# hannesweisbach/channelcoding

Measured on AMD Instinct MI355X. Metric: decoded frames/sec (coded bits/sec = value x 255), BCH(255,231) min-sum, batch=2^20, higher is better.
Workload: dtype f32

## Files before the change

channelcoding_amd/csrc/cc_internal.hpp:

```cpp
#pragma once
#include <hip/hip_runtime.h>

#include <cstdint>
#include <memory>
#include <mutex>
#include <string>
#include <vector>

#include "../../include/channelcoding_amd.h"
#include "galois.hpp"

namespace ccamd {

struct MinSumGeometry {
  int W = 64, C = 4, frames_per_wave = 1, KW = 1;
};

struct MinSumParams {
  int n, K, KW;
  int variant;
  int stop_rule;
  unsigned iterations;
  float alpha_f;
  float beta_f;
// ... 41 lines not shown
  uint32_t root_log[64] = {0};
  uint32_t n = 0, k = 0, l = 0, t = 0, nroots = 0, q = 0;
  uint32_t nf = 0;
  int family = 0;
};

}

namespace ccamd {
struct McWorkspace;
void mc_workspace_free(McWorkspace *w);
struct HostStage;
void host_stage_free(HostStage *s);
}

struct cc_code {
  cc_desc desc;
  int device = 0;
  std::unique_ptr<ccamd::Field> field;
  ccamd::CodeTables tab;
  bool wide = false;
  std::unique_ptr<ccamd::FieldT<uint16_t>> field16;
  ccamd::CodeTablesT<uint16_t> tab16;
  ccamd::WideTables wide_dev;
  uint16_t *d_wide = nullptr;
  bool soft = false;
  std::vector<uint8_t> custom_H;
  bool matrix_only = false;
  unsigned ms_rows = 0;
  ccamd::MinSumGeometry geo;
  uint32_t *d_colmask = nullptr;
  uint16_t *d_diag = nullptr;
  uint32_t *d_colbits = nullptr;
  uint8_t *d_parity = nullptr;
  ccamd::AlgebraicTables *d_alg = nullptr;
  ccamd::AlgebraicTables h_alg;
  mutable ccamd::McWorkspace *mc = nullptr;
  mutable ccamd::HostStage *stage = nullptr;
  mutable std::mutex lazy_lock;
  hipMemPool_t pool = nullptr;
  int num_cus = 256;
  bool force_generic = false;
  std::string name;
  bool shortened = false;
  unsigned long long *d_osd_rows = nullptr;
};

namespace ccamd {

inline bool rs_twisted(const cc_code *code) {
  return code->tab.family == CC_FAMILY_RS && (code->desc.mu != 1 || code->desc.step != 1);
}

inline hipError_t workspace_alloc(const cc_code *code, void **p, size_t bytes, hipStream_t stream) {
  return code->pool ? hipMallocFromPoolAsync(p, bytes, code->pool, stream) : hipMallocAsync(p, bytes, stream);
}

struct Scratch {
  const cc_code *code;
  hipStream_t stream;
  void *p[6] = {nullptr, nullptr, nullptr, nullptr, nullptr, nullptr};
  int used = 0;
  Scratch(const cc_code *c, hipStream_t s) : code(c), stream(s) {}
  Scratch(const Scratch &) = delete;
  Scratch &operator=(const Scratch &) = delete;
  ~Scratch() {
    for (int i = 0; i < used; ++i)
      if (p[i]) (void)hipFreeAsync(p[i], stream);
  }
  template <class T>
  hipError_t get(T **out, size_t bytes) {
    const hipError_t e = workspace_alloc(code, &p[used], bytes ? bytes : 1, stream);
    *out = static_cast<T *>(p[used]);
    if (e == hipSuccess) ++used;
    return e;
  }
};

void set_last_error(const std::string &s);
int hip_fail(hipError_t e, const char *what);

#define CC_HIP_TRY(expr)                                   \
  do {                                                     \
    hipError_t _e = (expr);                                \
    if (_e != hipSuccess) return ccamd::hip_fail(_e, #expr); \
  } while (0)

int launch_minsum(const cc_code *code, const float *d_llr, const uint16_t *d_er, const uint32_t *d_er_off,
                  uint8_t *d_hard, float *d_L, uint16_t *d_iters, int32_t *d_status, size_t B, hipStream_t stream);
struct DiagGeometry {
  unsigned n, k, w;
  int D, LPF, CPL;
  bool scms;
  int np = 0;
  int gap[4] = {0, 0, 0, 0};
};
const DiagGeometry *diag_geometry(const CodeTables &t);
std::vector<uint16_t> build_diag_table(const CodeTables &t, int D, int W, int np = 0, const int *gap = nullptr);
size_t minsum_diag_lds_bytes(const DiagGeometry &g);
MinSumParams minsum_params(const cc_code *code);
bool minsum_shortcuts_enabled();
bool minsum_diag_supported(const cc_code *code);
int launch_minsum_diag_compact(const cc_code *code, uint32_t *d_ctl, uint32_t *d_pool, unsigned cap, const float *d_llr,
                               uint8_t *d_hard, uint16_t *d_iters, int32_t *d_status, hipStream_t stream);
std::string minsum_diag_name(const cc_code *code);
int launch_minsum_diag(const cc_code *code, const MinSumParams &p, const float *d_llr, const uint16_t *d_er,
                       const uint32_t *d_er_off, uint8_t *d_hard, float *d_L, uint16_t *d_iters, int32_t *d_status,
                       size_t B, hipStream_t stream);
bool algebraic_long_needed(const cc_code *code, bool erasures);
int launch_algebraic_long(const cc_code *code, bool float_in, const void *d_in, const uint16_t *d_er,
                          const uint32_t *d_er_off, uint8_t *d_out, int32_t *d_nerr, int32_t *d_status, size_t B,
                          hipStream_t stream);
int launch_algebraic(const cc_code *code, bool float_in, const void *d_in, const uint16_t *d_er,
                     const uint32_t *d_er_off, uint8_t *d_out, int32_t *d_nerr, int32_t *d_status, size_t B,
                     hipStream_t stream);
bool algebraic_chunk_supported(const cc_code *code, bool erasures);
int launch_algebraic_chunk(const cc_code *code, bool float_in, const void *d_in, const uint16_t *d_er,
                           const uint32_t *d_er_off, uint8_t *d_out, int32_t *d_nerr, int32_t *d_status, size_t B,
                           hipStream_t stream, int il = 1);
int launch_chase(const cc_code *code, const float *d_llr, unsigned p, uint8_t *d_out, int32_t *d_nerr, float *d_metric,
                 int32_t *d_status, size_t B, hipStream_t stream);
int chase_frames_per_wave(const cc_code *code, unsigned p, bool soft, bool extended = false);
int launch_chase_soft(const cc_code *code, const float *d_llr, unsigned p, float beta, uint8_t *d_out, float *d_ext,
                      int32_t *d_nerr, float *d_metric, int32_t *d_status, size_t B, hipStream_t stream);
int launch_chase_extended(const cc_code *code, const float *d_llr, unsigned p, float beta, uint8_t *d_out, float *d_ext,
                          int32_t *d_nerr, float *d_metric, int32_t *d_status, size_t B, hipStream_t stream);
int launch_osd(const cc_code *code, const float *d_llr, unsigned order, uint8_t *d_out, int32_t *d_nerr, float *d_metric,
               int32_t *d_status, size_t B, hipStream_t stream);
int osd_frames_per_wave(const cc_code *code);
std::vector<unsigned long long> build_osd_rows(const CodeTables &t);
int launch_gmd(const cc_code *code, const uint8_t *d_words, const float *d_rel, unsigned m, uint8_t *d_out, int32_t *d_nerr,
               float *d_metric, int32_t *d_status, size_t B, hipStream_t stream);
bool bitslice_supported(const cc_code *code);
int launch_bitslice_syndromes(const cc_code *code, bool float_in, const void *d_in, uint8_t *d_out, uint8_t *d_synd, size_t B,
                              hipStream_t stream, int il = 1);
bool bitslice_encode_supported(const cc_code *code);
int launch_bitslice_encode(const cc_code *code, const uint8_t *d_msg, uint8_t *d_cw, size_t B, hipStream_t stream, int il = 1);
int launch_bitslice_chien(const void *d_lamp, void *d_masks, size_t B, bool long_locators, hipStream_t stream);
int launch_bitslice_roots_transpose(const void *d_masks, void *d_rootsT, size_t B, hipStream_t stream);
constexpr uint32_t kLogZero = 512;
int launch_chunk_bm(const cc_code *code, const uint8_t *d_synd, const uint16_t *d_er, const uint32_t *d_er_off,
                    uint16_t *d_llg, uint16_t *d_meta, unsigned long long *d_mask, uint8_t *d_lamp, int ncoef,
                    uint32_t *d_nleft, int32_t *d_nerr, int32_t *d_status, size_t B, hipStream_t stream);
int algebraic_route(const cc_code *code, size_t B, bool erasures);
bool planes_small_call(const cc_code *code, size_t B);
int launch_pgz_erasures(const cc_code *code, const uint8_t *d_in, const uint16_t *d_er, const uint32_t *d_er_off,
                        uint8_t *d_out, int32_t *d_nerr, int32_t *d_status, size_t B, hipStream_t stream);
constexpr int diag_variant_part(int variant, int parts) {
  const int order = variant == CC_ALG_MS ? 0 : variant == CC_ALG_NMS ? 1 : variant == CC_ALG_OMS ? 2
                  : variant == CC_ALG_SCMS2 ? 3 : variant == CC_ALG_SCMS1 ? 4 : 5;
  return order % parts;
}

enum DiagRowBody { DIAG_ROWS_BUTTERFLY = 0, DIAG_ROWS_FOUR = 1, DIAG_ROWS_FOUR_PIPELINED = 2 };
#ifndef CC_DIAG_FOUR_ROW_BODY
#define CC_DIAG_FOUR_ROW_BODY 1
#endif
constexpr int diag_row_body(int K, int D, int LPF, int variant) {
  const bool plain = variant == CC_ALG_MS || variant == CC_ALG_NMS || variant == CC_ALG_OMS || variant == CC_ALG_2DNMS;
  return (K == 24 && D == 7 && LPF == 16 && plain) ? CC_DIAG_FOUR_ROW_BODY : DIAG_ROWS_BUTTERFLY;
}

int launch_wide_correct(const cc_code *code, const uint16_t *d_in, const uint16_t *d_er, const uint32_t *d_off,
                        uint16_t *d_out, int32_t *d_nerr, int32_t *d_status, size_t B, hipStream_t stream);
int launch_wide_pgz_erasures(const cc_code *code, const uint16_t *d_in, const uint16_t *d_er, const uint32_t *d_off,
                        uint16_t *d_out, int32_t *d_nerr, int32_t *d_status, size_t B, hipStream_t stream);
int launch_wide_encode(const cc_code *code, const uint16_t *d_msg, uint16_t *d_cw, size_t B, hipStream_t stream);
int launch_wide_extract(const cc_code *code, const uint16_t *d_cw, uint16_t *d_msg, size_t B, hipStream_t stream);
std::vector<uint8_t> build_parity_table(const Field &f, const CodeTables &t);
int launch_encode(const cc_code *code, const uint8_t *d_msg, uint8_t *d_cw, size_t B, hipStream_t stream);
int launch_encode_bits(const cc_code *code, const uint8_t *d_msg, uint8_t *d_cw, size_t B, hipStream_t stream);
int launch_extract(const cc_code *code, const uint8_t *d_cw, uint8_t *d_msg, size_t B, hipStream_t stream);
int launch_pack_bits(const void *d_sym, int width, size_t n, uint8_t *d_packed, size_t B, hipStream_t stream);
int launch_unpack_bits(const uint8_t *d_packed, size_t n, void *d_sym, int width, size_t B, hipStream_t stream);
bool packed_native_supported(const cc_code *code, size_t B);
int launch_packed_correct(const cc_code *code, const uint8_t *d_in, uint8_t *d_out, int32_t *d_nerr, int32_t *d_status,
                          size_t B, hipStream_t stream);
bool packed_long_supported(const cc_code *code, size_t B);
int launch_packed_long_correct(const cc_code *code, const uint8_t *d_in, uint8_t *d_out, int32_t *d_nerr, int32_t *d_status,
                               size_t B, hipStream_t stream);
bool packed_encode_native(const cc_code *code);
bool packed_extract_native(const cc_code *code);
int launch_packed_encode(const cc_code *code, const uint8_t *d_msg, uint8_t *d_cw, size_t B, hipStream_t stream);
int launch_packed_extract(const cc_code *code, const uint8_t *d_cw, uint8_t *d_msg, size_t B, hipStream_t stream);
constexpr size_t kInterleaveMax = 256;
constexpr size_t kInterleaveNativeMax = 16;
int launch_interleave(const void *d_in, int width, size_t n, size_t I, void *d_out, size_t B, bool to_interleaved,
                      hipStream_t stream);
bool interleaved_native_supported(const cc_code *code, size_t B, size_t I, bool erasures);
bool interleaved_encode_native(const cc_code *code, size_t I);
bool interleaved_extract_native(const cc_code *code, size_t I);
int launch_interleaved_extract(const cc_code *code, const void *d_cw, void *d_msg, size_t B, size_t I, hipStream_t stream);
struct ProductShape {
  int e;
  size_t w1, w2, k1, k2, N;
};
ProductShape product_shape(const cc_product *pc);
size_t product_chunk_blocks(size_t N, size_t blocks, size_t at_least = 1);
int launch_product_decode(const cc_product *pc, const float *d_y, uint8_t *d_out, float *d_ext, int32_t *d_status, size_t B,
                          hipStream_t stream);
int launch_product_encode(const cc_product *pc, const uint8_t *d_msg, uint8_t *d_cw, size_t B, hipStream_t stream);
int launch_product_extract(const cc_product *pc, const uint8_t *d_cw, uint8_t *d_msg, size_t B, hipStream_t stream);
int product_awgn(const cc_product *pc, double ebno_db, uint64_t seed, uint64_t first_block, size_t blocks,
                 int random_codewords, float *d_y, uint8_t *d_sent, hipStream_t stream);
int mc_run_product(const cc_product *pc, double ebno_db, uint64_t seed, uint64_t first_block, size_t blocks,
                   int random_codewords, uint64_t *d_counters, hipStream_t stream);
int mc_run_product_hard(const cc_product *pc, double ebno_db, uint64_t seed, uint64_t first_block, size_t blocks,
                        int random_codewords, uint64_t *d_counters, hipStream_t stream);
int launch_product_hard(const cc_product *pc, const uint8_t *d_in, uint8_t *d_out, int32_t *d_nflip, int32_t *d_last,
                        int32_t *d_status, size_t B, hipStream_t stream);
struct StaircaseShape {
  int e;
  size_t m, r, kb, L, N, K;
};
StaircaseShape staircase_shape(const cc_staircase *sc);
size_t staircase_lds_bytes(const cc_staircase *sc);
int launch_staircase_decode(const cc_staircase *sc, const uint8_t *d_in, uint8_t *d_out, int32_t *d_nflip, int32_t *d_status,
                            size_t B, hipStream_t stream);
int launch_staircase_encode(const cc_staircase *sc, const uint8_t *d_msg, uint8_t *d_cw, size_t B, hipStream_t stream);
int launch_staircase_extract(const cc_staircase *sc, const uint8_t *d_cw, uint8_t *d_msg, size_t B, hipStream_t stream);
int staircase_awgn(const cc_staircase *sc, double ebno_db, uint64_t seed, uint64_t first_stream, size_t streams,
                   int random_codewords, uint8_t *d_z, uint8_t *d_sent, hipStream_t stream);
int mc_run_staircase(const cc_staircase *sc, double ebno_db, uint64_t seed, uint64_t first_stream, size_t streams,
                     int random_codewords, uint64_t *d_counters, hipStream_t stream);
int mc_run(cc_code *code, double ebno_db, uint64_t seed, uint64_t first_frame, size_t frames, int random_codewords,
           uint64_t *d_counters, hipStream_t stream);
int mc_run_chase(cc_code *code, unsigned p, double ebno_db, uint64_t seed, uint64_t first_frame, size_t frames,
                 int random_codewords, uint64_t *d_counters, hipStream_t stream);
int mc_run_osd(cc_code *code, unsigned order, double ebno_db, uint64_t seed, uint64_t first_frame, size_t frames,
               int random_codewords, uint64_t *d_counters, hipStream_t stream);
int mc_run_gmd(cc_code *code, unsigned m, double ebno_db, uint64_t seed, uint64_t first_frame, size_t frames,
               int random_codewords, uint64_t *d_counters, hipStream_t stream);
int mc_awgn_symbols(cc_code *code, double ebno_db, uint64_t seed, uint64_t first_frame, size_t frames, int random_codewords,
                    uint8_t *d_words, float *d_rel, uint8_t *d_sent, hipStream_t stream);
int mc_awgn(cc_code *code, double ebno_db, uint64_t seed, uint64_t first_frame, size_t frames, int random_codewords,
            float *d_llr, uint8_t *d_sent, hipStream_t stream);
int launch_awgn_values(const cc_code *code, int n, float sigma, uint64_t seed, uint64_t first_frame, size_t frames,
                       float *d_llr, const uint8_t *sent, hipStream_t stream, unsigned long long *d_counters = nullptr);
int launch_awgn_hard(const cc_code *code, int n, float sigma, uint64_t seed, uint64_t first_frame, size_t frames,
                     uint8_t *d_hard, const uint8_t *sent, hipStream_t stream, unsigned long long *d_counters = nullptr);
int launch_random_bits(const cc_code *code, int l, uint64_t seed, uint64_t first_frame, size_t frames, uint8_t *d_msg,
                       hipStream_t stream);
int mc_run_discrete(cc_code *code, double p_error, double p_erasure, uint64_t seed, uint64_t first_frame, size_t frames,
                    int random_codewords, uint64_t *d_counters, hipStream_t stream);
int mc_discrete(cc_code *code, double p_error, double p_erasure, uint64_t seed, uint64_t first_frame, size_t frames,
                int random_codewords, uint8_t *d_recv, uint16_t *d_erasures, uint32_t *d_erasure_offsets,
                uint8_t *d_sent, hipStream_t stream);
int mc_run_burst(cc_code *code, const cc_burst_channel &ch, uint64_t seed, uint64_t first_frame, size_t frames,
                 int random_codewords, uint64_t *d_counters, hipStream_t stream);
int mc_burst(cc_code *code, const cc_burst_channel &ch, uint64_t seed, uint64_t first_frame, size_t frames,
             int random_codewords, uint8_t *d_recv, uint8_t *d_sent, uint8_t *d_state, hipStream_t stream);
int mc_run_burst_erasure(cc_code *code, const cc_burst_channel &ch, const cc_burst_detector &det, uint64_t seed,
                         uint64_t first_frame, size_t frames, int random_codewords, uint64_t *d_counters,
                         hipStream_t stream);
int mc_burst_erasure(cc_code *code, const cc_burst_channel &ch, const cc_burst_detector &det, uint64_t seed,
                     uint64_t first_frame, size_t frames, int random_codewords, uint8_t *d_recv, uint8_t *d_sent,
                     uint8_t *d_state, uint8_t *d_flag, uint16_t *d_erasures, uint32_t *d_erasure_offsets,
                     hipStream_t stream);
int mc_run_bsc_packed(cc_code *code, double p_error, uint64_t seed, uint64_t first_frame, size_t frames,
                      int random_codewords, uint64_t *d_counters, hipStream_t stream);
int mc_bsc_packed(cc_code *code, double p_error, uint64_t seed, uint64_t first_frame, size_t frames, int random_codewords,
                  uint8_t *d_recv, uint8_t *d_sent, hipStream_t stream);
int launch_bsc_packed(const cc_code *code, unsigned long long threshold, uint64_t seed, uint64_t first_frame, size_t frames,
                      const uint8_t *d_sent, uint8_t *d_recv, unsigned long long *d_counters, hipStream_t stream);
int launch_random_packed_messages(const cc_code *code, uint64_t seed, uint64_t first_frame, size_t frames, uint8_t *d_msg,
                                  hipStream_t stream);
int launch_count_packed(const cc_code *code, const uint8_t *d_decoded, const uint8_t *d_sent, const int32_t *d_status,
                        size_t frames, unsigned long long *d_counters, hipStream_t stream);
int packed_correct_route(const cc_code *code, const uint8_t *d_in, uint8_t *d_out, int32_t *d_nerr, int32_t *d_status,
                         size_t B, hipStream_t stream);
int packed_encode_route(const cc_code *code, const uint8_t *d_msg, uint8_t *d_cw, size_t B, hipStream_t stream);
int minsum_kernel_info(const cc_code *code, std::string &name, uint32_t &frames_per_wg, uint32_t &threads,
                       uint32_t &lds);

}
```

channelcoding_amd/csrc/minsum_diag.hip:

```cpp
#include "minsum_diag_impl.hpp"

#include <algorithm>
#include <cstdlib>

namespace ccamd {

using DiagLaunch = int (*)(const cc_code *, const MinSumParams &, const float *, const uint16_t *, const uint32_t *,
                           uint8_t *, float *, uint16_t *, int32_t *, size_t, hipStream_t);
#define CC_PART_DECL(NAME, I)                                                                                        \
  int launch_minsum_diag_##NAME##_p##I(const cc_code *, const MinSumParams &, const float *, const uint16_t *,       \
                                       const uint32_t *, uint8_t *, float *, uint16_t *, int32_t *, size_t, hipStream_t);
#define CC_PARTS_1(M, NAME) M(NAME, 0)
#define CC_PARTS_2(M, NAME) CC_PARTS_1(M, NAME) M(NAME, 1)
#define CC_PARTS_3(M, NAME) CC_PARTS_2(M, NAME) M(NAME, 2)
#define CC_PARTS_6(M, NAME) CC_PARTS_3(M, NAME) M(NAME, 3) M(NAME, 4) M(NAME, 5)
#define GEO(NAME, N, KK, W, DD, LL, CC, OO, SC, PA, LK, PP) CC_PARTS_##PP(CC_PART_DECL, NAME)
#include "minsum_diag_geos.inc"
#undef GEO
namespace {
struct DiagEntry {
  DiagGeometry geo;
  int parts;
  DiagLaunch launch[6];
};
// ... 41 lines not shown
    bool ok = true;
    for (int p = 0; p < np && ok; ++p) {
      std::vector<unsigned> c;
      for (unsigned s : sup)
        if (in_sup[s + gap[p]]) c.push_back(s);
      for (size_t i = c.size(); i > 1; --i) std::swap(c[i - 1], c[next() % i]);
      bool res[16] = {false};
      for (int pass = 0; pass < 2 && low[p].size() < static_cast<size_t>(W); ++pass)
        for (unsigned s : c) {
          if (used[s] || used[s + gap[p]] || (pass == 0 && res[s % 16])) continue;
          used[s] = used[s + gap[p]] = 1;
          res[s % 16] = true;
          low[p].push_back(s);
          if (low[p].size() == static_cast<size_t>(W)) break;
        }
      ok = low[p].size() == static_cast<size_t>(W);
    }
    if (!ok) continue;
    std::vector<unsigned> single;
    for (unsigned s : sup)
      if (!used[s]) single.push_back(s);
    int cost = 0;
    for (int p = 0; p < np; ++p) cost += passes(low[p]);
    {
      int cnt[16] = {0}, mx = 0;
      for (unsigned s : single) mx = std::max(mx, ++cnt[s % 16]);
      cost += std::max(singles_per_lane, mx);
    }
    if (cost < best_cost) {
      best_cost = cost;
      best_low = low;
      best_single = single;
    }
  }
  if (best_cost == 1 << 30) return {};
  std::vector<uint16_t> out(static_cast<size_t>(D) * W, 0xFFFFu);
  for (int p = 0; p < np; ++p) {
    std::sort(best_low[p].begin(), best_low[p].end());
    for (int l = 0; l < W; ++l) {
      out[(2 * p) * W + l] = static_cast<uint16_t>(best_low[p][l]);
      out[(2 * p + 1) * W + l] = static_cast<uint16_t>(best_low[p][l] + gap[p]);
    }
  }
  std::vector<std::vector<unsigned>> cls(16);
  for (unsigned s : best_single) cls[s % 16].push_back(s);
  std::vector<std::vector<unsigned>> slot(singles_per_lane);
  int turn = 0;
  for (int r = 0; r < 16; ++r)
    for (unsigned s : cls[r]) {
      int tries = 0;
      while (slot[turn % singles_per_lane].size() >= static_cast<size_t>(W) && tries++ < singles_per_lane) ++turn;
      slot[turn++ % singles_per_lane].push_back(s);
    }
  for (int g = 0; g < singles_per_lane; ++g)
    for (size_t l = 0; l < slot[g].size(); ++l) out[(2 * np + g) * W + l] = static_cast<uint16_t>(slot[g][l]);
  return out;
}

std::vector<uint16_t> build_diag_table(const CodeTables &t, int D, int W, int np, const int *gap) {
#ifdef CC_AMD_EXPERIMENTS
  if (const char *e = std::getenv("CC_AMD_EXP_FAKE_DEAL"); e && e[0] == '1') {
    std::vector<uint16_t> out(static_cast<size_t>(D) * W);
    for (int d = 0; d < D; ++d)
      for (int l = 0; l < W; ++l)
        out[d * W + l] = static_cast<uint16_t>(d < 2 * np ? l + W * (d & ~1) + (d & 1) : l + W * d);
    return out;
  }
#endif
  if (np > 0) return build_paired_table(t, D, W, np, gap);
  std::vector<std::vector<unsigned>> cls(W);
  for (unsigned s : t.row0_support) cls[s % W].push_back(s);
  std::vector<std::vector<unsigned>> grp(D);
  std::vector<unsigned> left;
  for (int r = 0; r < W; ++r)
    for (size_t e = 0; e < cls[r].size(); ++e) {
      if (e < static_cast<size_t>(D))
        grp[e].push_back(cls[r][e]);
      else
        left.push_back(cls[r][e]);
    }
  for (int g = 0; g < D; ++g) {
    while (grp[g].size() < static_cast<size_t>(W) && !left.empty()) {
      size_t best = 0;
      int best_mult = 1 << 30;
      for (size_t c = 0; c < left.size(); ++c) {
        int mult = 1;
        for (unsigned s : grp[g]) mult += (s % W == left[c] % W);
        if (mult < best_mult) {
          best_mult = mult;
          best = c;
        }
      }
      grp[g].push_back(left[best]);
      left.erase(left.begin() + static_cast<long>(best));
    }
  }
  for (int g = 0; g + 1 < D; ++g)
    while (grp[g].size() < static_cast<size_t>(W) && !grp[D - 1].empty()) {
      grp[g].push_back(grp[D - 1].back());
      grp[D - 1].pop_back();
    }
  const size_t real_last = grp[D - 1].size();
  auto group_cost = [&](const std::vector<unsigned> &g) {
    int cnt[16] = {0}, mx = 0, sq = 0;
    for (unsigned s : g) ++cnt[s % 16];
    for (int c : cnt) {
      mx = c > mx ? c : mx;
      sq += c * c;
    }
    return mx * 1000 + sq;
  };
  bool improved = true;
  while (improved) {
    improved = false;
    for (int a = 0; a < D && !improved; ++a)
      for (int b = a + 1; b < D && !improved; ++b)
        for (size_t x = 0; x < grp[a].size() && !improved; ++x)
          for (size_t y = 0; y < grp[b].size() && !improved; ++y) {
            const int before = group_cost(grp[a]) + group_cost(grp[b]);
            std::swap(grp[a][x], grp[b][y]);
            if (group_cost(grp[a]) + group_cost(grp[b]) < before)
              improved = true;
            else
              std::swap(grp[a][x], grp[b][y]);
          }
  }
  std::vector<uint16_t> out(static_cast<size_t>(D) * W, 0xFFFFu);
  for (int g = 0; g < D; ++g)
    for (size_t l = 0; l < grp[g].size(); ++l) out[g * W + l] = static_cast<uint16_t>(grp[g][l]);
  (void)real_last;
  return out;
}

bool minsum_diag_supported(const cc_code *code) {
  if (code->d_diag == nullptr || code->desc.iterations == 0) return false;
  const int alg = code->desc.algorithm;
  const DiagGeometry *geo = diag_geometry(code->tab);
  if (!geo) return false;
  if (alg == CC_ALG_SCMS1) return true;
  if (alg == CC_ALG_SCMS2) return geo->scms;
  if (alg != CC_ALG_MS && alg != CC_ALG_NMS && alg != CC_ALG_OMS && alg != CC_ALG_2DNMS) return false;
  if (alg == CC_ALG_OMS && !(code->desc.beta >= 0.0)) return false;
  const float a = static_cast<float>(code->desc.alpha);
  if ((alg == CC_ALG_NMS || alg == CC_ALG_2DNMS) && !(a == a && a - a == 0.0f)) return false;
  return diag_geometry(code->tab) != nullptr;
}


std::string minsum_diag_name(const cc_code *code) {
  const DiagGeometry *g = diag_geometry(code->tab);
  if (!g) return "minsum_diag_kernel";
  const int body = diag_row_body(static_cast<int>(g->k), g->D, g->LPF, code->desc.algorithm);
  return "minsum_diag_kernel<K=" + std::to_string(g->k) + ",D=" + std::to_string(g->D) + ",LPF=" + std::to_string(g->LPF) +
         (body == DIAG_ROWS_FOUR_PIPELINED ? ",four-row-pipelined>" : body == DIAG_ROWS_FOUR ? ",four-row>" : ",row-pipelined>");
}

size_t minsum_diag_lds_bytes(const DiagGeometry &g) {
  const bool partial = g.w != static_cast<unsigned>(g.LPF * g.D);
  const size_t fpw = 64 / g.LPF, rc = static_cast<size_t>(g.LPF) * g.CPL + (partial ? 48 : (g.LPF == 8 && g.CPL == 8 ? 8 : 16));
  return 4 * (fpw * rc * 8 + (fpw / 2) * rc * 8) + 256 * 4 +
         4 * static_cast<size_t>(g.CPL) * 256;
}


namespace {

__global__ void __launch_bounds__(256)
twopass_gather_kernel(const uint32_t *__restrict__ ctl, unsigned sample, unsigned cap, const uint32_t *__restrict__ list,
                      const float *__restrict__ llr, float *__restrict__ llr2, int n) {
  if (!two_pass_in_effect(ctl, sample, cap)) return;
  const unsigned long long cnt = ctl[1];
  const int lane = threadIdx.x & 63;
  const unsigned long long nwaves = static_cast<unsigned long long>(gridDim.x) * 4;
  for (unsigned long long k = static_cast<unsigned long long>(blockIdx.x) * 4 + (threadIdx.x >> 6); k < cnt; k += nwaves) {
    const float *src = llr + static_cast<unsigned long long>(list[k]) * n;
    float *dst = llr2 + k * n;
    for (int j = lane; j < n; j += 64) dst[j] = src[j];
  }
}
__global__ void __launch_bounds__(256)
twopass_scatter_kernel(const uint32_t *__restrict__ ctl, unsigned sample, unsigned cap, const uint32_t *__restrict__ list,
                       const uint8_t *__restrict__ hard2, const uint16_t *__restrict__ iters2,
                       const int32_t *__restrict__ status2, uint8_t *__restrict__ hard, uint16_t *__restrict__ iters,
                       int32_t *__restrict__ status, int n) {
  if (!two_pass_in_effect(ctl, sample, cap)) return;
  const unsigned long long cnt = ctl[1];
  const int lane = threadIdx.x & 63;
  const unsigned long long nwaves = static_cast<unsigned long long>(gridDim.x) * 4;
  for (unsigned long long k = static_cast<unsigned long long>(blockIdx.x) * 4 + (threadIdx.x >> 6); k < cnt; k += nwaves) {
    const unsigned long long f = list[k];
    for (int j = lane; j < n; j += 64) hard[f * n + j] = hard2[k * n + j];
    if (lane == 0) {
      if (iters) iters[f] = iters2[k];
      if (status) status[f] = status2[k];
    }
  }
}

bool two_pass_enabled() { return minsum_shortcuts_enabled(); }

int launch_two_pass(const cc_code *code, const DiagEntry *e, const MinSumParams &p, const float *d_llr, uint8_t *d_hard,
                    uint16_t *d_iters, int32_t *d_status, size_t B, hipStream_t stream) {
  const size_t n = code->tab.n, cap = B / 4, sample = 4096;
  auto up = [](size_t v) { return (v + 255) & ~static_cast<size_t>(255); };
  constexpr size_t max_runs = 4, o_pool = 256, pool_bytes = POOL_WORDS * 4;
  const size_t o_list = o_pool + (max_runs + 2) * pool_bytes, o_llr = o_list + up(cap * 4), o_hard = o_llr + up(cap * n * 4),
               o_it = o_hard + up(cap * n), o_st = o_it + up(cap * 2), total = o_st + up(cap * 4);
  uint8_t *ws = nullptr;
  CC_HIP_TRY(workspace_alloc(code, reinterpret_cast<void **>(&ws), total, stream));
  uint32_t *ctl = reinterpret_cast<uint32_t *>(ws), *list = reinterpret_cast<uint32_t *>(ws + o_list);
  float *llr2 = reinterpret_cast<float *>(ws + o_llr);
  uint8_t *hard2 = ws + o_hard;
  uint16_t *it2 = reinterpret_cast<uint16_t *>(ws + o_it);
  int32_t *st2 = reinterpret_cast<int32_t *>(ws + o_st);
  int rc = CC_OK;
  hipError_t he = hipMemsetAsync(ctl, 0, o_list, stream);
  if (he != hipSuccess) rc = hip_fail(he, "two-pass control words");
  MinSumParams q = p;
  q.ctl = ctl;
  q.list = list;
  q.list_cap = static_cast<unsigned>(cap);
  constexpr unsigned den = 8;
  q.sample = static_cast<unsigned>(sample * 8 / den);
  q.first_pass = 2;
  const size_t runs = B >= 16 * sample ? max_runs : 1, per = sample / runs, hop = (B / runs) & ~static_cast<size_t>(63);
  for (size_t r = 0; r < runs && rc == CC_OK; ++r) {
    const size_t at = r * hop;
    q.pool = reinterpret_cast<uint32_t *>(ws + o_pool + r * pool_bytes);
    rc = launcher(e, q)(code, q, d_llr + at * n, nullptr, nullptr, d_hard + at * n, nullptr, d_iters ? d_iters + at : nullptr,
                        d_status ? d_status + at : nullptr, per, stream);
  }
  if (rc == CC_OK) {
    q.first_pass = 1;
    q.gate = 1;
    q.pool = reinterpret_cast<uint32_t *>(ws + o_pool + max_runs * pool_bytes);
    rc = launcher(e, q)(code, q, d_llr, nullptr, nullptr, d_hard, nullptr, d_iters, d_status, B, stream);
  }
  if (rc == CC_OK) {
    const int grid = code->num_cus * 4;
    const unsigned su = q.sample, cu = q.list_cap;
    hipLaunchKernelGGL(twopass_gather_kernel, dim3(grid), dim3(256), 0, stream, ctl, su, cu, list, d_llr, llr2,
                       static_cast<int>(n));
    q.first_pass = 0;
    q.gate = -1;
    q.dual = 1;
    q.pool = reinterpret_cast<uint32_t *>(ws + o_pool + (max_runs + 1) * pool_bytes);
    q.llr2 = llr2;
    q.hard2 = hard2;
    q.iters2 = it2;
    q.status2 = st2;
    rc = launcher(e, q)(code, q, d_llr, nullptr, nullptr, d_hard, nullptr, d_iters, d_status, B, stream);
    if (rc == CC_OK)
      hipLaunchKernelGGL(twopass_scatter_kernel, dim3(grid), dim3(256), 0, stream, ctl, su, cu, list, hard2, it2, st2,
                         d_hard, d_iters, d_status, static_cast<int>(n));
  }
  if (rc == CC_OK) {
    he = hipGetLastError();
    if (he != hipSuccess) rc = hip_fail(he, "two-pass kernels launch");
  }
  (void)hipFreeAsync(ws, stream);
  return rc;
}

}

bool minsum_shortcuts_enabled() {
  static const bool v = [] {
    const char *e = std::getenv("CC_AMD_TWO_PASS");
    return !(e && e[0] == '0');
  }();
  return v;
}

int launch_minsum_diag_compact(const cc_code *code, uint32_t *d_ctl, uint32_t *d_pool, unsigned cap, const float *d_llr,
                               uint8_t *d_hard, uint16_t *d_iters, int32_t *d_status, hipStream_t stream) {
  const DiagEntry *e = diag_entry(code->tab);
  if (!e) return CC_ERR_UNSUPPORTED;
  MinSumParams q = minsum_params(code);
  q.ctl = d_ctl;
  q.pool = d_pool;
  q.sample = 1;
  q.list_cap = cap;
  q.gate = -1;
  q.dual = 1;
  q.llr2 = d_llr;
  q.hard2 = d_hard;
  q.iters2 = d_iters;
  q.status2 = d_status;
  return launcher(e, q)(code, q, d_llr, nullptr, nullptr, d_hard, nullptr, d_iters, d_status, cap, stream);
}

int launch_minsum_diag(const cc_code *code, const MinSumParams &p, const float *d_llr, const uint16_t *d_er,
                       const uint32_t *d_er_off, uint8_t *d_hard, float *d_L, uint16_t *d_iters, int32_t *d_status,
                       size_t B, hipStream_t stream) {
  const DiagEntry *e = diag_entry(code->tab);
  if (!e) return CC_ERR_UNSUPPORTED;
  const bool plain = p.variant == CC_ALG_MS || p.variant == CC_ALG_NMS || p.variant == CC_ALG_OMS || p.variant == CC_ALG_2DNMS;
  const double work = static_cast<double>(B) * code->tab.n * code->tab.k;
  if (two_pass_enabled() && plain && p.stop_rule != CC_STOP_AS_SHIPPED && p.iterations >= 2 && d_er_off == nullptr &&
      d_L == nullptr && work >= 1.5e9)
    return launch_two_pass(code, e, p, d_llr, d_hard, d_iters, d_status, B, stream);
  uint32_t *pool = nullptr;
  CC_HIP_TRY(workspace_alloc(code, reinterpret_cast<void **>(&pool), POOL_WORDS * 4, stream));
  int rc = CC_OK;
  const hipError_t he = hipMemsetAsync(pool, 0, POOL_WORDS * 4, stream);
  if (he != hipSuccess) rc = hip_fail(he, "frame pool");
  MinSumParams q = p;
// ... 8 lines not shown
```

channelcoding_amd/csrc/minsum_diag_impl.hpp:

```cpp
#pragma once
#include <cstdio>
#include <cstdlib>
#include <type_traits>
#include <utility>

#include "cc_internal.hpp"
#include "wave_ops.hpp"


namespace ccamd {
namespace {



template <int... Is, typename F>
__device__ __forceinline__ void static_for_impl(std::integer_sequence<int, Is...>, F &&f) {
  (f(std::integral_constant<int, Is>{}), ...);
}
template <int N, typename F>
__device__ __forceinline__ void static_for(F &&f) {
  static_for_impl(std::make_integer_sequence<int, N>{}, static_cast<F &&>(f));
}
template <int... Gs>
struct PairGaps {
// ... 279 lines not shown
  auto ordinal_frame = [&](unsigned o) -> unsigned long long {
    return static_cast<unsigned long long>(blockIdx.x) * GPW + (o % GPW) + static_cast<unsigned long long>(o / GPW) * ngroups;
  };
  auto take_frame = [&]() -> unsigned long long {
    unsigned o = 0;
    if (lam == 0) o = atomicAdd(&wg_next, 1u);
    o = static_cast<unsigned>(__builtin_amdgcn_ds_bpermute((lane & ~(LPF - 1)) * 4, static_cast<int>(o)));
    return ordinal_frame(o);
  };
  unsigned long long frame, nextf;
  if constexpr (POOL) {
    const unsigned ofr = (blockIdx.x / S) * GPW + wid * FPW + fl;
    if (lam == 0) my_ords = make_uint2(ofr, ofr + Ws * GPW);
    frame = frame_of(ofr);
    nextf = frame_of(ofr + Ws * GPW);
  } else {
    frame = (static_cast<unsigned long long>(blockIdx.x) * 4 + wid) * FPW + fl;
    nextf = frame + ngroups;
  }
  bool active = frame < B;
  unsigned it = 0;
  constexpr bool NEEDQ = (VARIANT == CC_ALG_SCMS1 || VARIANT == CC_ALG_SCMS2);
  constexpr bool QONLY = !SINGLE && ((VARIANT == CC_ALG_SCMS2 && 2 * K * D + 64 > 256) ||
                                     (VARIANT == CC_ALG_SCMS1 && K * D >= 160 && OCC >= 2));
  constexpr bool KEEPQ = (VARIANT == CC_ALG_SCMS2 && !SINGLE) || QONLY;
  float R[(SINGLE || QONLY) ? 1 : K][(SINGLE || QONLY) ? 1 : D];
  float Q[KEEPQ ? K : 1][KEEPQ ? D : 1];
  __shared__ uint2 row_state[QONLY ? 4 * FPW * K : 1];
  uint2 *const my_rows = row_state + (QONLY ? (wid * FPW + fl) * K : 0);
  uint2 rsq = make_uint2(0u, 0u);
  constexpr bool BITS1 = VARIANT == CC_ALG_SCMS1 && !SINGLE && !QONLY;
  constexpr int RPW = 32 / D;
  constexpr int NW = (K + RPW - 1) / RPW;
  uint32_t SW[BITS1 ? NW : 1], ZW[BITS1 ? NW : 1];

  constexpr bool X4 = (LPF * CPL - 1) >= 4 * LPF;
  constexpr int NF = (LPF * CPL - 1) / (4 * LPF);
  auto stage = [&](unsigned long long f) {
    if (f < B) {
      const float *src = llr + f * n;
      if constexpr (X4) {
        const float *v = src + 4 * lam;
        const float *vt = v + (n - 4 * LPF);
        uint32_t m0_save;
        const uint32_t sb = __builtin_amdgcn_readfirstlane(stg_lds);
        static_assert(NF == 1 || NF == 3, "x4 staging is written out for one or three aligned copies");
        if constexpr (NF == 3) {
          asm volatile(
              "s_mov_b32 %0, m0\n\ts_mov_b32 m0, %3\n\ts_nop 0\n\tglobal_load_lds_dwordx4 %1, off\n\t"
              "s_add_u32 m0, %3, %4\n\ts_nop 0\n\tglobal_load_lds_dwordx4 %1, off offset:%7\n\t"
              "s_add_u32 m0, %3, %5\n\ts_nop 0\n\tglobal_load_lds_dwordx4 %1, off offset:%8\n\t"
              "s_add_u32 m0, %3, %6\n\ts_nop 0\n\tglobal_load_lds_dwordx4 %2, off\n\ts_mov_b32 m0, %0"
              : "=&s"(m0_save)
              : "v"(v), "v"(vt), "s"(sb), "n"(1024 - LPF * 16), "n"(2048 - 2 * LPF * 16), "n"(3072), "n"(LPF * 16),
                "n"(2 * LPF * 16)
              : "memory", "scc");
        } else {
          asm volatile(
              "s_mov_b32 %0, m0\n\ts_mov_b32 m0, %3\n\ts_nop 0\n\tglobal_load_lds_dwordx4 %1, off\n\t"
              "s_add_u32 m0, %3, 1024\n\ts_nop 0\n\tglobal_load_lds_dwordx4 %2, off\n\ts_mov_b32 m0, %0"
              : "=&s"(m0_save)
              : "v"(v), "v"(vt), "s"(sb)
              : "memory", "scc");
        }
      } else {
#pragma unroll
        for (int c = 0; c < CPL; ++c) {
          const int j = lam + LPF * c;
          if (j < n) {
            uint32_t m0_save;
            asm volatile("s_mov_b32 %0, m0\n\ts_mov_b32 m0, %2\n\ts_nop 0\n\tglobal_load_lds_dword %1, off\n\ts_mov_b32 m0, %0"
                         : "=&s"(m0_save) : "v"(src + j), "s"(stg_lds + c * 256) : "memory");
          }
        }
      }
    }
  };
  const char *stg_full = stg + fl * LPF * 16 + lam * 4;
  const char *stg_tail = stg + NF * 1024 + fl * LPF * 16 + (lam - n + 4 * LPF) * 4;
  auto staged = [&](int c) -> float {
    if constexpr (X4) {
      if (c < 4 * NF) return *reinterpret_cast<const float *>(stg_full + (c / 4) * 1024 + (c % 4) * 4 * LPF);
      return *reinterpret_cast<const float *>(stg_tail + 4 * LPF * c);
    } else {
      return *reinterpret_cast<const float *>(stg + c * 256 + lane * 4);
    }
  };
  auto setup = [&](unsigned long long f) {
#pragma unroll
    for (int c = 0; c < CPL; ++c) {
      float y = staged(c) + 0.0f;
      if (c == CPL - 1 && lam + LPF * c >= n) y = 0.0f;
      *reinterpret_cast<float2 *>(cy_base + (col0 + LPF * c) * 8) = make_cell(0.0f, y);
    }
    if (er_off != nullptr) {
      for (uint32_t e = er_off[f]; e < er_off[f + 1]; ++e) {
        const int pos = er[e];
        if ((pos & (LPF - 1)) == lam) *reinterpret_cast<float *>(cy_base + (fl * RC + pos) * 8 + y_off) = 0.0f;
      }
    }
    if constexpr (!SINGLE && !QONLY) static_for<K>([&](auto I) { static_for<D>([&](auto Dd) { R[I][Dd] = 0.0f; }); });
    if constexpr (KEEPQ) static_for<K>([&](auto I) { static_for<D>([&](auto Dd) { Q[I][Dd] = 0.0f; }); });
    if constexpr (QONLY)
      for (int r = lam; r < K; r += LPF) my_rows[r] = make_uint2(0u, 0u);
    if constexpr (BITS1) static_for<NW>([&](auto Wd) { SW[Wd] = 0u; ZW[Wd] = 0xFFFFFFFFu; });
  };

#pragma unroll
  for (int c = 0; c < CPL; ++c)
    if constexpr (!SINGLE) *reinterpret_cast<float *>(cn_lane + (col0 + LPF * c) * 8) = 0.0f;
  if (active) {
    stage(frame);
    asm volatile("s_waitcnt vmcnt(0)" ::: "memory");
    setup(frame);
    stage(nextf);
    if (POOL && PREDRAW && lam == 0) opd = draw();
  }

  while (__any(active)) {
    constexpr bool PREFETCH = !(BITS1 && K * D >= 160) && !SINGLE;
    constexpr bool TRED = BODY != DIAG_ROWS_BUTTERFLY;
    static_assert(!TRED || (LPF == 16 && K % 4 == 0 && !SINGLE && !NEEDQ),
                  "four rows per reduction: a frame per DPP row, whole row groups, plain variants (the self-correcting ones spill)");
    constexpr bool READY = TRED && VARIANT == CC_ALG_MS;
    constexpr bool EARLY_PF = TRED && PREFETCH;
    float2 cyq[D];
    float2 carry_cy[NLK ? NLK : 1];
    float carry_sum[NLK ? NLK : 1];
    auto fetch = [&](auto IC) {
      constexpr int row = decltype(IC)::value;
      if constexpr (QONLY) rsq = my_rows[row];
      static_for<D>([&](auto DD) {
        constexpr int d = TRED ? D - 1 - DD : DD;
        if constexpr (d < 2 * NLK && (d & 1) == 0 && row >= 1) {
          cyq[d] = carry_cy[d / 2];
          return;
        }
#ifdef CC_EXP_NO_CYR
        asm volatile("" : "=v"(cyq[d].x), "=v"(cyq[d].y));
#else
#ifdef CC_EXP_O0_B32
        if constexpr (SINGLE) {
          const int at = aCY[slot_base<PG>(d)] + 8 * (row + slot_gap<PG>(d));
          cyq[d].x = *reinterpret_cast<const float *>(cy_base + at + (4 - y_off));
          cyq[d].y = *reinterpret_cast<const float *>(cy_base + at + y_off);
          return;
        }
#endif
        cyq[d] = *reinterpret_cast<const float2 *>(cy_base + aCY[slot_base<PG>(d)] + 8 * (row + slot_gap<PG>(d)));
#endif
      });
    };
    float Tloc[D];
    auto row_front = [&](auto IR, uint32_t &o1, uint32_t &o2, uint32_t &os) {
      constexpr int i = decltype(IR)::value;
      if constexpr (!PREFETCH) fetch(IR);
      [[maybe_unused]] auto wget = [&](auto DD) -> float {
        if constexpr (SINGLE) return Tloc[DD];
        else if constexpr (QONLY) return Q[i][DD];
        else return R[i][DD];
      };
      auto wset = [&](auto DD, float v) {
        if constexpr (SINGLE) Tloc[DD] = v;
        else if constexpr (!QONLY) R[i][DD] = v;
      };
      [[maybe_unused]] const float old_hi = u2f(rsq.y & 0x7FFFFFFFu);
      [[maybe_unused]] uint32_t old_Y = (rsq.x ^ rsq.y);
      if constexpr (QONLY) asm volatile("" : "+v"(old_Y));
      {
        float a1 = 0.0f, a2 = (D == 1) ? 3.402823466e+38f : 0.0f;
        uint32_t s = 0;
        uint32_t qs[D];
        float mag[D], qv[D];
        uint32_t keep = 0;
        constexpr int wi = BITS1 ? i / RPW : 0, sh = BITS1 ? (i % RPW) * D : 0;
        if constexpr (BITS1) {
          uint32_t tw = 0, tz = 0;
          static_for<D>([&](auto DD) {
            constexpr int d = DD;
            const float t = (cyq[d].x - R[i][d]) + cyq[d].y;
            R[i][d] = t;
            tw = __builtin_amdgcn_alignbit(tw, f2u(t), 31);
            tz = shift_in_is_zero(tz, t);
          });
          constexpr uint32_t field = ((D == 32 ? 0u : (1u << D)) - 1u) << sh;
          const uint32_t tws = tw << sh, tzs = tz << sh;
          keep = ZW[wi] | ~(SW[wi] ^ tws);
          SW[wi] = (SW[wi] & ~field) | (tws & keep);
          ZW[wi] = (ZW[wi] & ~field) | ((~keep & field) | tzs);
        }
        static_for<D>([&](auto DD) {
          constexpr int d = DD;
          float q;
          if constexpr (BITS1) {
            const int32_t m = __builtin_amdgcn_sbfe(static_cast<int32_t>(keep), sh + D - 1 - d, 1);
            q = u2f(f2u(R[i][d]) & static_cast<uint32_t>(m));
          } else if constexpr (SINGLE) {
            q = cell_y(cyq[d]);
            if constexpr (NEEDQ) q = self_correct<VARIANT>(q, 0.0f);
          } else {
            float r_old;
            if constexpr (QONLY) r_old = u2f(f2u(__builtin_amdgcn_fmed3f(Q[i][d], -old_hi, old_hi)) ^ old_Y);
            else r_old = R[i][d];
            float e = cyq[d].x - r_old;
            if constexpr (VARIANT == CC_ALG_2DNMS) e = __fmul_rn(p.beta_f, e);
            q = e + cyq[d].y;
            if constexpr (QONLY && VARIANT == CC_ALG_SCMS1) {
              const uint32_t so = f2u(Q[i][d]), st = f2u(q);
              const int differ = static_cast<int>(so ^ st) >> 31;
              const uint32_t zero_old = umin32(so, 1u) - 1u;
              q = u2f(static_cast<uint32_t>(__builtin_amdgcn_bitop3_b32(static_cast<int>(st), static_cast<int>(zero_old), differ,
                                                                        0xD0)));
              Q[i][d] = q;
            } else if constexpr (KEEPQ) {
              q = self_correct<VARIANT>(q, Q[i][d]);
              Q[i][d] = q;
            }
          }
          wset(DD, q);
          qv[d] = q;
        });
        if constexpr (EARLY_PF) {
          static_for<NLK>([&](auto P) { carry_cy[P] = cyq[2 * P + 1]; });
          asm volatile("" ::: "memory");
          if constexpr (i + 1 < K) fetch(std::integral_constant<int, i + 1>{});
          asm volatile("" ::: "memory");
        }
        static_for<D>([&](auto DD) {
          constexpr int d = DD;
          const float q = qv[d];
          float a = __builtin_fabsf(q);
          uint32_t qb = f2u(q);
          if constexpr (PARTIAL && d == D - 1) {
            a = __builtin_fmaxf(a, pen);
            qb &= sgn_keep;
          }
          qs[d] = qb;
          constexpr bool RAW = (SINGLE || BITS1) && !PARTIAL && D >= 2;
          mag[d] = RAW ? q : a;
          if constexpr (D == 2 && d == 1) {
            a2 = RAW ? max_abs2(mag[0], mag[1]) : __builtin_fmaxf(mag[0], mag[1]);
            a1 = RAW ? min_abs2(mag[0], mag[1]) : __builtin_fminf(mag[0], mag[1]);
          } else if constexpr (d == 0 && D == 1) {
            a1 = a;
          } else if constexpr (d == 2) {
            a2 = RAW ? med3_abs3(mag[0], mag[1], mag[2]) : __builtin_amdgcn_fmed3f(mag[0], mag[1], mag[2]);
            a1 = RAW ? min3_abs3(mag[0], mag[1], mag[2]) : __builtin_fminf(__builtin_fminf(mag[0], mag[1]), mag[2]);
          } else if constexpr (d >= 4 && (d & 1) == 0) {
            const float md = RAW ? med3_abs23(a1, mag[d - 1], mag[d]) : __builtin_amdgcn_fmed3f(a1, mag[d - 1], mag[d]);
            a1 = RAW ? min3_abs23(a1, mag[d - 1], mag[d]) : __builtin_fminf(__builtin_fminf(a1, mag[d - 1]), mag[d]);
            a2 = __builtin_fminf(a2, md);
          } else if constexpr (d == D - 1 && d >= 3 && (d & 1) == 1) {
            a2 = RAW ? med3_abs1(a1, mag[d], a2) : __builtin_amdgcn_fmed3f(a1, mag[d], a2);
            a1 = RAW ? min_abs1(a1, mag[d]) : __builtin_fminf(a1, mag[d]);
          }
        });
        s = qs[0];
        static_for<(D - 1) / 2>([&](auto T) {
          s = static_cast<uint32_t>(__builtin_amdgcn_bitop3_b32(static_cast<int>(s), static_cast<int>(qs[1 + 2 * T]),
                                                                static_cast<int>(qs[2 + 2 * T]), 0x96));
        });
        if constexpr ((D - 1) % 2) s ^= qs[D - 1];
        o1 = f2u(a1);
        o2 = f2u(a2);
        os = s;
      }
      if constexpr (!EARLY_PF) {
        static_for<NLK>([&](auto P) { carry_cy[P] = cyq[2 * P + 1]; });
        if constexpr (PREFETCH && i + 1 < K) fetch(std::integral_constant<int, i + 1>{});
      }
    };
    auto row_cn = [&](auto IR, float (&cn)[D]) {
      constexpr int i = decltype(IR)::value;
      static_for<D>([&](auto DD) {
        constexpr int d = DD;
        if constexpr (d < 2 * NLK && (d & 1) == 0 && i >= 1)
          cn[d] = carry_sum[d / 2];
        else if constexpr (SINGLE)
          cn[d] = cell_cs(cyq[d]);
        else
#ifdef CC_EXP_NO_CNR
          asm volatile("" : "=v"(cn[d]));
#else
          cn[d] = *reinterpret_cast<const float *>(cn_lane + aCY[slot_base<PG>(d)] + 8 * (i + slot_gap<PG>(d)));
#endif
      });
    };
    auto row_back = [&](auto IR, uint32_t m1v, uint32_t m2v, uint32_t sg0, float (&cn)[D]) {
      constexpr int i = decltype(IR)::value;
      float rt[QONLY ? D : 1];
      bool made = false;
      (void)made;
      [[maybe_unused]] auto wget = [&](auto DD) -> float {
        if constexpr (SINGLE) return Tloc[DD];
        else if constexpr (QONLY) return made ? rt[DD] : Q[i][DD];
        else return R[i][DD];
      };
      auto wset = [&](auto DD, float v) {
        if constexpr (SINGLE) Tloc[DD] = v;
        else if constexpr (QONLY) rt[DD] = v;
        else R[i][DD] = v;
      };
      if constexpr (!READY) asm volatile("" : "+v"(sg0));
      const uint32_t sign31 = sg0 & 0x80000000u;
      if constexpr (VARIANT == CC_ALG_MS || VARIANT == CC_ALG_SCMS1 || VARIANT == CC_ALG_SCMS2) {
        uint32_t Y = READY ? m1v : (m1v ^ m2v) | sign31;
#ifndef CC_EXP_BITOP3_POST
        asm volatile("" : "+v"(Y));
#endif
        const float hi = u2f(m2v);
        static_for<D>([&](auto DD) {
          wset(DD, u2f(f2u(__builtin_amdgcn_fmed3f(wget(DD), -hi, hi)) ^ Y));
        });
      } else {
        const uint32_t H1 = f2u(horizontal<VARIANT>(u2f(m1v), p.alpha_f, p.beta_d));
        const uint32_t H2 = f2u(horizontal<VARIANT>(u2f(m2v), p.alpha_f, p.beta_d));
        static_for<D>([&](auto DD) {
          const uint32_t mag = (__builtin_fabsf(wget(DD)) == u2f(m1v)) ? H2 : H1;
          wset(DD, u2f(xad(mag, sign31, f2u(wget(DD)) & 0x80000000u)));
        });
      }
      made = true;
      if constexpr (QONLY) {
        if (lam == 0) my_rows[i] = make_uint2(m1v, m2v | sign31);
      }
      float sum[D];
      static_for<D>([&](auto DD) {
        constexpr int d = D - 1 - DD;
        sum[d] = cn[d] + wget(std::integral_constant<int, d>{});
      });
      __builtin_amdgcn_sched_barrier(0);
      static_for<D>([&](auto DD) {
        constexpr int d = DD;
        if constexpr (d < 2 * NLK && (d & 1) == 1 && i + 1 < K)
          carry_sum[d / 2] = sum[d];
        else if constexpr (SINGLE)
          *reinterpret_cast<float *>(cy_base + aWR[slot_base<PG>(d)] + 8 * (i + slot_gap<PG>(d))) = sum[d];
        else
#ifdef CC_EXP_NO_CNW
          asm volatile("" ::"v"(sum[d]));
#else
          *reinterpret_cast<float *>(cn_lane + aCY[slot_base<PG>(d)] + 8 * (i + slot_gap<PG>(d))) = sum[d];
#endif
      });
      asm volatile("" ::: "memory");
    };
    if constexpr (PREFETCH) fetch(std::integral_constant<int, 0>{});
    if constexpr (TRED) {
      constexpr int NG = K / 4;
      uint32_t ZA[NG], ZB[NG], ZC[READY ? 1 : NG];
      auto fronts = [&](auto IG) {
        constexpr int g = decltype(IG)::value;
        uint32_t a1[4], a2[4], sg[4];
        static_for<4>([&](auto J) { row_front(std::integral_constant<int, 4 * g + J>{}, a1[J], a2[J], sg[J]); });
        uint32_t z1, z2, zs;
        transposed_reduce4(a1, a2, sg, z1, z2, zs);
        if constexpr (READY) {
          ZA[g] = (z1 ^ z2) | (zs & 0x80000000u);
          ZB[g] = z2;
        } else {
          ZA[g] = z1;
          ZB[g] = z2;
          ZC[g] = zs;
        }
      };
      auto backs = [&](auto IG) {
        constexpr int g = decltype(IG)::value;
        static_for<4>([&](auto J) {
          float cn[D];
          row_cn(std::integral_constant<int, 4 * g + J>{}, cn);
          const uint32_t b0 = bank_bcast<J>(ZA[g]), b1 = bank_bcast<J>(ZB[g]);
          uint32_t b2 = 0;
          if constexpr (!READY) b2 = bank_bcast<J>(ZC[g]);
          row_back(std::integral_constant<int, 4 * g + J>{}, b0, b1, b2, cn);
        });
      };
      if constexpr (BODY == DIAG_ROWS_FOUR_PIPELINED) {
        fronts(std::integral_constant<int, 0>{});
        static_for<NG>([&](auto IG) {
          if constexpr (IG + 1 < NG) fronts(std::integral_constant<int, IG + 1>{});
          backs(IG);
        });
      } else {
        static_for<NG>([&](auto IG) {
          fronts(IG);
          backs(IG);
        });
      }
    } else {
      static_for<K>([&](auto IR) {
        uint32_t m1[1], m2[1], sg[1];
        row_front(IR, m1[0], m2[0], sg[0]);
        float cn[D];
        row_cn(IR, cn);
#ifndef CC_EXP_NO_REDUCE
        row_allreduce<1, LPF>(m1, m2, sg);
#endif
        row_back(IR, m1[0], m2[0], sg[0], cn);
      });
    }

    uint32_t acc = 0;
    auto stop_scan = [&](auto ORC) {
      float cnv[CPL], yc[CPL];
      uint32_t cb[CPL];
#pragma unroll
      for (int c = 0; c < CPL; ++c) {
        if constexpr (SINGLE) {
          const float2 cy = *reinterpret_cast<const float2 *>(cy_base + (col0 + LPF * c) * 8);
          cnv[c] = cy.x;
          yc[c] = cy.y;
        } else {
          cnv[c] = *reinterpret_cast<const float *>(cn_lane + (col0 + LPF * c) * 8);
          yc[c] = *reinterpret_cast<const float *>(cy_base + (col0 + LPF * c) * 8 + 4);
        }
        cb[c] = cbits[lam + LPF * c];
      }
      asm volatile("" ::: "memory");
#pragma unroll
      for (int c = 0; c < CPL; ++c) {
        const int m = static_cast<int>(f2u(cnv[c] + yc[c])) >> 31;
        if constexpr (decltype(ORC)::value)
          acc = static_cast<uint32_t>(__builtin_amdgcn_bitop3_b32(static_cast<int>(acc), m, static_cast<int>(cb[c]), 0xF8));
        else
          acc = static_cast<uint32_t>(__builtin_amdgcn_bitop3_b32(static_cast<int>(acc), m, static_cast<int>(cb[c]), 0x78));
      }
      if constexpr (!SINGLE) {
#pragma unroll
        for (int c = 0; c < CPL; ++c) {
          *reinterpret_cast<float *>(cy_base + (col0 + LPF * c) * 8) = cnv[c];
          *reinterpret_cast<float *>(cn_lane + (col0 + LPF * c) * 8) = 0.0f;
        }
      }
    };
    bool ok;
    if (SINGLE && p.stop_rule == CC_STOP_AS_SHIPPED) {
      ok = true;
    } else if (p.stop_rule == CC_STOP_PUBLISHED) {
      stop_scan(std::true_type{});
      ok = group_or<LPF>(acc) == 0;
    } else {
      stop_scan(std::false_type{});
      ok = (p.stop_rule == CC_STOP_AS_SHIPPED) || group_xor<LPF>(acc) == 0;
    }
#ifdef CC_EXP_NEVER_STOP
    ok = false;
#endif
    const bool finished = SINGLE || ok || (it + 1 >= p.iterations);
    if (finished && active) {
      const uint2 od = POOL ? my_ords : make_uint2(0u, 0u);
      const unsigned long long done = POOL ? frame_of(od.x) : frame;
      const unsigned done_it = ok ? it : p.iterations;
      frame = POOL ? frame_of(od.y) : nextf;
      active = frame < B;
      uint8_t *hp = hard + done * n + lam;
      float *Lp = Lout ? Lout + done * n + lam : nullptr;
      const bool handed = SINGLE && p.first_pass != 0 && !ok;
      auto emit = [&](int c, float L) {
        if (handed) return;
        if (c < CPL - 1 || lam + LPF * c < n) {
          hp[LPF * c] = (L < 0.0f) ? 1 : 0;
          if (Lp) Lp[LPF * c] = L;
        }
      };
      if (active) {
        asm volatile("s_waitcnt vmcnt(0)" ::: "memory");
#pragma unroll
        for (int c = 0; c < CPL; ++c) {
          const float2 cy = *reinterpret_cast<const float2 *>(cy_base + (col0 + LPF * c) * 8);
          float y = staged(c) + 0.0f;
          if (c == CPL - 1 && lam + LPF * c >= n) y = 0.0f;
          *reinterpret_cast<float2 *>(cy_base + (col0 + LPF * c) * 8) = make_cell(0.0f, y);
          emit(c, cy.x + cy.y);
        }
        if (er_off != nullptr) {
          for (uint32_t e = er_off[frame]; e < er_off[frame + 1]; ++e) {
            const int pos = er[e];
            if ((pos & (LPF - 1)) == lam) *reinterpret_cast<float *>(cy_base + (fl * RC + pos) * 8 + y_off) = 0.0f;
          }
        }
        if constexpr (!SINGLE && !QONLY) static_for<K>([&](auto I) { static_for<D>([&](auto Dd) { R[I][Dd] = 0.0f; }); });
        if constexpr (KEEPQ) static_for<K>([&](auto I) { static_for<D>([&](auto Dd) { Q[I][Dd] = 0.0f; }); });
        if constexpr (QONLY)
          for (int r = lam; r < K; r += LPF) my_rows[r] = make_uint2(0u, 0u);
        if constexpr (BITS1) static_for<NW>([&](auto Wd) { SW[Wd] = 0u; ZW[Wd] = 0xFFFFFFFFu; });
        it = 0;
      } else {
#pragma unroll
        for (int c = 0; c < CPL; ++c) {
          const float2 cy = *reinterpret_cast<const float2 *>(cy_base + (col0 + LPF * c) * 8);
          emit(c, cy.x + cy.y);
        }
      }
      if (lam == 0) {
        if (handed) {
          if (p.first_pass == 2) {
            atomicAdd(&p.ctl[2], 1u);
          } else {
            const uint32_t at = atomicAdd(&p.ctl[1], 1u);
            if (at < p.list_cap) p.list[at] = static_cast<uint32_t>(done);
            else p.ctl[3] = 1u;
          }
        } else {
          if (iters_out) iters_out[done] = static_cast<uint16_t>(done_it);
          if (status_out) status_out[done] = ok ? CC_FRAME_OK : CC_FRAME_NOT_CONVERGED;
        }
      }
      if (active) {
        if constexpr (POOL) {
          if (!PREDRAW && lam == 0) opd = draw();
          const unsigned nx = drawn(opd);
          stage(frame_of(nx));
          if (lam == 0) {
            my_ords = make_uint2(od.y, nx);
            if (PREDRAW) opd = draw();
          }
        } else {
          nextf = take_frame();
          stage(nextf);
        }
      }
    } else {
      ++it;
    }
  }
  asm volatile("s_waitcnt vmcnt(0)" ::: "memory");
}

}

namespace {

template <int K, int D, int LPF, int CPL, int OCC, bool SCMS = false, bool PARTIAL = false, typename PG = PairGaps<>,
          bool CHAIN = false, int PARTS = 1, int PART = 0>
int launch_diag_geometry(const cc_code *code, const MinSumParams &p, const float *d_llr, const uint16_t *d_er,
                         const uint32_t *d_er_off, uint8_t *d_hard, float *d_L, uint16_t *d_iters, int32_t *d_status,
                         size_t B, hipStream_t stream) {
  constexpr int RB = 1;
  constexpr bool Q_ONLY_2 = 2 * K * D + 64 > 256, Q_ONLY_1 = K * D >= 160 && OCC >= 2;
  constexpr int OCC_S = Q_ONLY_2 ? OCC : (2 * K * D + 64 <= 128) ? 4 : (2 * K * D + 64 <= 168) ? 3 : 2;
  constexpr int FPW = 64 / LPF;
  if (!(code->tab.n > static_cast<unsigned>(LPF * (CPL - 1)) && code->tab.n <= static_cast<unsigned>(LPF * CPL))) {
    set_last_error("minsum_diag: only the last owned column of a lane may lie beyond the frame");
    return CC_ERR_UNSUPPORTED;
  }
// ... 68 lines not shown
```

Measured before the change: 71.29 million.

## Interleave next row-group fronts with current group backs in diag min-sum

Adds a zipped four-row body that runs the back-half (check-node update and write) of each row in group g inside the front-half of the matching row in group g+1. Each back step is fenced with sched_barrier, and the next row's check-node values are loaded right after each back. It becomes the default body for the K=24, D=7, LPF=16 geometry, replacing the plain four-row body. The aim is to hide the latency of the LDS and transposed reduction behind independent work, at the cost of higher register pressure and a more rigid instruction schedule.

New measurement: 72.26 million (median of 6 runs). +1.4%, better.

```diff
diff --git a/channelcoding_amd/csrc/cc_internal.hpp b/channelcoding_amd/csrc/cc_internal.hpp
--- a/channelcoding_amd/csrc/cc_internal.hpp
+++ b/channelcoding_amd/csrc/cc_internal.hpp
@@ -217,13 +217,15 @@
   return order % parts;
 }
 
-enum DiagRowBody { DIAG_ROWS_BUTTERFLY = 0, DIAG_ROWS_FOUR = 1, DIAG_ROWS_FOUR_PIPELINED = 2 };
-#ifndef CC_DIAG_FOUR_ROW_BODY
-#define CC_DIAG_FOUR_ROW_BODY 1
-#endif
+enum DiagRowBody { DIAG_ROWS_BUTTERFLY = 0, DIAG_ROWS_FOUR = 1, DIAG_ROWS_FOUR_PIPELINED = 2, DIAG_ROWS_FOUR_ZIPPED = 3 };
 constexpr int diag_row_body(int K, int D, int LPF, int variant) {
   const bool plain = variant == CC_ALG_MS || variant == CC_ALG_NMS || variant == CC_ALG_OMS || variant == CC_ALG_2DNMS;
-  return (K == 24 && D == 7 && LPF == 16 && plain) ? CC_DIAG_FOUR_ROW_BODY : DIAG_ROWS_BUTTERFLY;
+  if (!(K == 24 && D == 7 && LPF == 16 && plain)) return DIAG_ROWS_BUTTERFLY;
+#ifdef CC_DIAG_FOUR_ROW_BODY
+  return CC_DIAG_FOUR_ROW_BODY;
+#else
+  return DIAG_ROWS_FOUR_ZIPPED;
+#endif
 }
 
 int launch_wide_correct(const cc_code *code, const uint16_t *d_in, const uint16_t *d_er, const uint32_t *d_off,
diff --git a/channelcoding_amd/csrc/minsum_diag.hip b/channelcoding_amd/csrc/minsum_diag.hip
--- a/channelcoding_amd/csrc/minsum_diag.hip
+++ b/channelcoding_amd/csrc/minsum_diag.hip
@@ -217,7 +217,10 @@
   if (!g) return "minsum_diag_kernel";
   const int body = diag_row_body(static_cast<int>(g->k), g->D, g->LPF, code->desc.algorithm);
   return "minsum_diag_kernel<K=" + std::to_string(g->k) + ",D=" + std::to_string(g->D) + ",LPF=" + std::to_string(g->LPF) +
-         (body == DIAG_ROWS_FOUR_PIPELINED ? ",four-row-pipelined>" : body == DIAG_ROWS_FOUR ? ",four-row>" : ",row-pipelined>");
+         (body == DIAG_ROWS_FOUR_ZIPPED      ? ",four-row-zipped>"
+          : body == DIAG_ROWS_FOUR_PIPELINED ? ",four-row-pipelined>"
+          : body == DIAG_ROWS_FOUR           ? ",four-row>"
+                                             : ",row-pipelined>");
 }
 
 size_t minsum_diag_lds_bytes(const DiagGeometry &g) {
diff --git a/channelcoding_amd/csrc/minsum_diag_impl.hpp b/channelcoding_amd/csrc/minsum_diag_impl.hpp
--- a/channelcoding_amd/csrc/minsum_diag_impl.hpp
+++ b/channelcoding_amd/csrc/minsum_diag_impl.hpp
@@ -455,7 +455,7 @@
       });
     };
     float Tloc[D];
-    auto row_front = [&](auto IR, uint32_t &o1, uint32_t &o2, uint32_t &os) {
+    auto row_front = [&](auto IR, uint32_t &o1, uint32_t &o2, uint32_t &os, auto &&mid) {
       constexpr int i = decltype(IR)::value;
       if constexpr (!PREFETCH) fetch(IR);
       [[maybe_unused]] auto wget = [&](auto DD) -> float {
@@ -529,6 +529,7 @@
           if constexpr (i + 1 < K) fetch(std::integral_constant<int, i + 1>{});
           asm volatile("" ::: "memory");
         }
+        mid();
         static_for<D>([&](auto DD) {
           constexpr int d = DD;
           const float q = qv[d];
@@ -652,10 +653,12 @@
     if constexpr (TRED) {
       constexpr int NG = K / 4;
       uint32_t ZA[NG], ZB[NG], ZC[READY ? 1 : NG];
-      auto fronts = [&](auto IG) {
+      auto fronts = [&](auto IG, auto &&mid) {
         constexpr int g = decltype(IG)::value;
         uint32_t a1[4], a2[4], sg[4];
-        static_for<4>([&](auto J) { row_front(std::integral_constant<int, 4 * g + J>{}, a1[J], a2[J], sg[J]); });
+        static_for<4>([&](auto J) {
+          row_front(std::integral_constant<int, 4 * g + J>{}, a1[J], a2[J], sg[J], [&] { mid(J); });
+        });
         uint32_t z1, z2, zs;
         transposed_reduce4(a1, a2, sg, z1, z2, zs);
         if constexpr (READY) {
@@ -678,22 +681,43 @@
           row_back(std::integral_constant<int, 4 * g + J>{}, b0, b1, b2, cn);
         });
       };
-      if constexpr (BODY == DIAG_ROWS_FOUR_PIPELINED) {
-        fronts(std::integral_constant<int, 0>{});
+      auto alone = [](auto) {};
+      if constexpr (BODY == DIAG_ROWS_FOUR_ZIPPED) {
+        float cn[D];
+        auto back_step = [&](auto IG, auto J) {
+          constexpr int i = 4 * decltype(IG)::value + decltype(J)::value;
+          __builtin_amdgcn_sched_barrier(0);
+          const uint32_t b0 = bank_bcast<J>(ZA[IG]), b1 = bank_bcast<J>(ZB[IG]);
+          uint32_t b2 = 0;
+          if constexpr (!READY) b2 = bank_bcast<J>(ZC[IG]);
+          row_back(std::integral_constant<int, i>{}, b0, b1, b2, cn);
+          if constexpr (i + 1 < K) row_cn(std::integral_constant<int, i + 1>{}, cn);
+          asm volatile("" ::: "memory");
+          __builtin_amdgcn_sched_barrier(0);
+        };
+        fronts(std::integral_constant<int, 0>{}, alone);
+        row_cn(std::integral_constant<int, 0>{}, cn);
+        asm volatile("" ::: "memory");
+        static_for<NG - 1>([&](auto IG) {
+          fronts(std::integral_constant<int, IG + 1>{}, [&](auto J) { back_step(IG, J); });
+        });
+        static_for<4>([&](auto J) { back_step(std::integral_constant<int, NG - 1>{}, J); });
+      } else if constexpr (BODY == DIAG_ROWS_FOUR_PIPELINED) {
+        fronts(std::integral_constant<int, 0>{}, alone);
         static_for<NG>([&](auto IG) {
-          if constexpr (IG + 1 < NG) fronts(std::integral_constant<int, IG + 1>{});
+          if constexpr (IG + 1 < NG) fronts(std::integral_constant<int, IG + 1>{}, alone);
           backs(IG);
         });
       } else {
         static_for<NG>([&](auto IG) {
-          fronts(IG);
+          fronts(IG, alone);
           backs(IG);
         });
       }
     } else {
       static_for<K>([&](auto IR) {
         uint32_t m1[1], m2[1], sg[1];
-        row_front(IR, m1[0], m2[0], sg[0]);
+        row_front(IR, m1[0], m2[0], sg[0], [] {});
         float cn[D];
         row_cn(IR, cn);
 #ifndef CC_EXP_NO_REDUCE
```
